# DRL-Navigation/DDRL4NAV

Measured on NVIDIA B200. Metric: PPO learner samples/s & batched policy actions/s at 1/2/4/8 B200, higher is better.
Workload: dtype f32 (three tcgen05 kind::f16 products of scaled fp16 hi/lo splits, fp32 accumulate)

## Files before the change

### ddrl4nav_b200/csrc/tc3.cu

```cuda
#include <cuda.h>
#include <cuda_fp16.h>

#include <algorithm>
#include <cstdlib>
#include <cstring>
#include <mutex>
#include <vector>

#include "common.cuh"
#include "layer_ops.h"
#include "prep_kernels.cuh"
#include "tc_ptx.cuh"

namespace ddrl {

constexpr int T3_BM = 128;
constexpr int T3_BK = 64;
constexpr int T3_CHUNK = 4;

__device__ unsigned long long g_tc3_wait[96];
#ifdef TC3_TIMING
#define T3_T0 const long long _t0 = clock64()
#define T3_ACC(acc) acc += clock64() - _t0
#define T3_WAIT(bar, par, acc) do { T3_T0; mbar_wait(bar, par); T3_ACC(acc); } while (0)
// ... 61 lines not shown
      ".reg .pred p;\n"
      "setp.ne.b32 p, %4, 0;\n"
      "tcgen05.mma.cta_group::1.kind::f16 [%0], [%1], %2, %3, p;\n"
      "}" ::"r"(tmem_d), "r"(tmem_a), "l"(db), "r"(idesc), "r"(accumulate) : "memory");
}

__device__ __forceinline__ void umma_f16_ss(uint32_t tmem_d, uint64_t da, uint64_t db, uint32_t idesc, uint32_t accumulate) {
  asm volatile(
      "{\n"
      ".reg .pred p;\n"
      "setp.ne.b32 p, %4, 0;\n"
      "tcgen05.mma.cta_group::1.kind::f16 [%0], %1, %2, %3, p;\n"
      "}" ::"r"(tmem_d), "l"(da), "l"(db), "r"(idesc), "r"(accumulate) : "memory");
}

template <int BN>
struct T3Cfg {
  static constexpr int A_SUB = T3_BM * 128;
  static constexpr int A_BYTES = 2 * A_SUB;
  static constexpr int B_BYTES = BN * 128;
  static constexpr int STAGE_BYTES = A_BYTES + 2 * B_BYTES;
  static constexpr int STAGES = BN <= 32 ? 5 : (BN <= 64 ? 4 : 3);
  static constexpr bool FOLD = BN <= 64;
  static constexpr int SA = BN <= 32 ? 4 : (BN <= 64 ? 3 : 2);
  static constexpr int NEPI = BN <= 32 ? 4 : 8;
  static constexpr int NSG = BN <= 64 ? 2 : 1;
  static constexpr int EPI0 = 4 + 4 * NSG;
  static constexpr int THREADS = (EPI0 + NEPI) * 32;
  static constexpr int COLS = BN / (NEPI / 4);
  static constexpr int TM_MAIN0 = 0, TM_MAIN1 = FOLD ? 2 * BN : BN, TM_CORR = FOLD ? 4 * BN : 2 * BN, TM_A = FOLD ? 5 * BN : 3 * BN;
  static constexpr int TMEM_COLS = 512;
  static constexpr int NBARS = 2 * STAGES + SA + 7;
  static constexpr int STG_OFF = STAGES * STAGE_BYTES;
  static constexpr int BAR_OFF = STG_OFF + NEPI * 4096;
  static constexpr int BIAS_OFF = BAR_OFF + 256;
  static constexpr int SMEM = 1024 + BIAS_OFF + BN * 4;
  static_assert(NBARS * 8 + 16 <= 256, "barrier block");
  static_assert(SMEM <= 232448, "shared memory budget");
  static_assert(TM_A + SA * 64 <= 512, "TMEM budget");
  static_assert(STAGES > SA, "the stage barrier of K block it - SA releases TMEM slot it % SA");
};

template <int BN>
__global__ void __launch_bounds__(T3Cfg<BN>::THREADS, 1)
tc3_kernel(const __grid_constant__ CUtensorMap tmA, const __grid_constant__ CUtensorMap tmBhi,
           const __grid_constant__ CUtensorMap tmBlo, const __grid_constant__ CUtensorMap tmA2,
           const __grid_constant__ CUtensorMap tmC, const __grid_constant__ CUtensorMap tmC2,
           const __grid_constant__ CUtensorMap tmM, const __grid_constant__ CUtensorMap tmM2, Tc3Args g) {
  using Cfg = T3Cfg<BN>;
  constexpr int S = Cfg::STAGES, SA = Cfg::SA;
  extern __shared__ uint8_t smem_dyn[];
  uint8_t* smem = smem_dyn + ((1024u - (smem_u32(smem_dyn) & 1023u)) & 1023u);
  uint64_t* bars = reinterpret_cast<uint64_t*>(smem + Cfg::BAR_OFF);
  uint64_t* bar_full = bars;
  uint64_t* bar_empty = bars + S;
  uint64_t* bar_aready = bars + 2 * S;
  uint64_t* bar_mfull = bars + 2 * S + SA;
  uint64_t* bar_mfree = bar_mfull + 2;
  uint64_t* bar_cfull = bar_mfull + 4;
  uint64_t* bar_cfree = bar_mfull + 5;
  uint64_t* bar_mask = bar_mfull + 6;
  uint32_t* tmem_slot = reinterpret_cast<uint32_t*>(bars + Cfg::NBARS);
  const int warp = threadIdx.x >> 5, lane = threadIdx.x & 31;
  const TcTap& tp = g.tap;
  const bool tapA = tp.mode != 0;

  if (warp == 0 && lane == 0) {
    mbar_init(smem_u32(bar_mask), 1);
    for (int s = 0; s < S; ++s) { mbar_init(smem_u32(bar_full + s), 1); mbar_init(smem_u32(bar_empty + s), 2); }
    for (int a = 0; a < SA; ++a) mbar_init(smem_u32(bar_aready + a), 4);
    for (int b = 0; b < 2; ++b) { mbar_init(smem_u32(bar_mfull + b), 1); mbar_init(smem_u32(bar_mfree + b), Cfg::NEPI); }
    mbar_init(smem_u32(bar_cfull), 1);
    mbar_init(smem_u32(bar_cfree), Cfg::NEPI);
    asm volatile("fence.mbarrier_init.release.cluster;" ::: "memory");
  }
  if (warp == 2) {
    asm volatile("tcgen05.alloc.cta_group::1.sync.aligned.shared::cta.b32 [%0], %1;" ::"r"(smem_u32(tmem_slot)),
                 "r"((uint32_t)Cfg::TMEM_COLS) : "memory");
    asm volatile("tcgen05.relinquish_alloc_permit.cta_group::1.sync.aligned;" ::: "memory");
  }
  tc_fence_before();
  __syncthreads();
  tc_fence_after();
  const uint32_t tmem_base = *tmem_slot;

  const int total_tiles = g.m_tiles * g.n_tiles;
  const int tile_step = (int)gridDim.x, tile_first = (int)blockIdx.x;
  const int nkb = g.kb_total;
  const bool ps = g.presplit != 0;
  const bool odd_tail = tapA && !ps && (tp.nslices & 1);

  if (warp == 0) {
    uint32_t it = 0;
    T3_ROLE_BEGIN
    for (int tile = tile_first; tile < total_tiles; tile += tile_step) {
      const int mt = tile / g.n_tiles, nt = tile - mt * g.n_tiles;
      const int m0 = mt * T3_BM, n0 = nt * BN;
      int b0 = 0, y0 = 0;
      const bool ph2 = tapA && mt >= tp.tiles1;
      if (tapA) {
        if (!ph2) { b0 = (mt / tp.tpi) * tp.nb; y0 = (mt % tp.tpi) * tp.ny * tp.sy - tp.py; }
        else { b0 = (mt - tp.tiles1) * tp.nb2; y0 = tp.y2 * tp.sy - tp.py; }
      }
      int cc = 0, kw = 0, kh = 0;
      for (int i = 0; i < nkb; ++i, ++it) {
        const uint32_t s = it % S;
        T3_WAITL(smem_u32(bar_empty + s), ((it / S) & 1) ^ 1, w0);
        const bool load_b = !g.b_resident || it < (uint32_t)S;
        const uint32_t b_tx = load_b ? 2u * Cfg::B_BYTES : 0u;
        if (elect_one()) {
          const uint32_t full = smem_u32(bar_full + s);
          const uint32_t a_dst = smem_u32(smem) + s * Cfg::STAGE_BYTES, bh_dst = a_dst + Cfg::A_BYTES, bl_dst = bh_dst + Cfg::B_BYTES;
          const int k = i * T3_BK;
          if (ps) {
            if (!tapA) {
              mbar_expect_tx(full, Cfg::A_BYTES + b_tx);
              tma_load_2d(&tmA, full, a_dst, k, m0);
              tma_load_2d(&tmM, full, a_dst + Cfg::A_SUB, k, m0);
            } else {
              const uint32_t box = (uint32_t)(ph2 ? tp.rows2 : tp.rows) * 128u;
              mbar_expect_tx(full, 2u * box + b_tx);
              tma_load_4d(ph2 ? &tmA2 : &tmA, full, a_dst, tp.c_off + cc * 64, kw - tp.px, y0 + kh, b0);
              tma_load_4d(ph2 ? &tmM2 : &tmM, full, a_dst + Cfg::A_SUB, tp.c_off + cc * 64, kw - tp.px, y0 + kh, b0);
            }
          } else if (!tapA) {
            mbar_expect_tx(full, Cfg::A_BYTES + b_tx);
            tma_load_2d(&tmA, full, a_dst, k, m0);
            tma_load_2d(&tmA, full, a_dst + Cfg::A_SUB, k + 32, m0);
          } else {
            const bool two = !(odd_tail && i == nkb - 1);
            const uint32_t box = (uint32_t)(ph2 ? tp.rows2 : tp.rows) * 128u;
            mbar_expect_tx(full, (two ? 2u : 1u) * box + b_tx);
            tma_load_4d(ph2 ? &tmA2 : &tmA, full, a_dst, tp.c_off + cc * 32, kw - tp.px, y0 + kh, b0);
            if (two) {
              int cc2 = cc + 1, kw2 = kw, kh2 = kh;
              if (cc2 == tp.cpb) { cc2 = 0; if (++kw2 == tp.KW) { kw2 = 0; ++kh2; } }
              tma_load_4d(ph2 ? &tmA2 : &tmA, full, a_dst + Cfg::A_SUB, tp.c_off + cc2 * 32, kw2 - tp.px, y0 + kh2, b0);
            }
          }
          if (load_b) {
            tma_load_2d(&tmBhi, full, bh_dst, k, n0);
            tma_load_2d(&tmBlo, full, bl_dst, k, n0);
          }
        }
        __syncwarp();
        if (tapA) {
#pragma unroll
          for (int j = 0; j < 2; ++j) {
            if (ps && j == 1) break;
            if (++cc == tp.cpb) { cc = 0; if (++kw == tp.KW) { kw = 0; ++kh; } }
          }
        }
      }
    }
    T3_ROLE_END(0, true);
  } else if (warp == 1 || warp == 3) {
    const bool chunk_role = warp == 1;
    const uint32_t idesc = (1u << 4) | ((uint32_t)(BN >> 3) << 17) | ((uint32_t)(T3_BM >> 4) << 24);
    const uint32_t idesc2 = (1u << 4) | ((uint32_t)((2 * BN) >> 3) << 17) | ((uint32_t)(T3_BM >> 4) << 24);
    const uint32_t smem_base = smem_u32(smem);
    const uint32_t t_corr = tmem_base + Cfg::TM_CORR;
    uint32_t it = 0, ch = 0, tl = 0;
    T3_ROLE_BEGIN
    for (int tile = tile_first; tile < total_tiles; tile += tile_step, ++tl) {
      for (int i = 0; i < nkb; ++i, ++it) {
        const uint32_t s = it % S, a = it % SA;
        const uint32_t buf = ch & 1;
        const bool first_in_chunk = (i % T3_CHUNK) == 0;
        const bool last_in_chunk = (i % T3_CHUNK) == T3_CHUNK - 1 || i == nkb - 1;
        const int ksteps = (odd_tail && i == nkb - 1) ? 2 : 4;
        if (chunk_role) { if (first_in_chunk) T3_WAIT(smem_u32(bar_mfree + buf), ((ch >> 1) & 1) ^ 1, w0); }
        else if (i == 0) T3_WAIT(smem_u32(bar_cfree), (tl & 1) ^ 1, w0);
        if (ps) T3_WAIT(smem_u32(bar_full + s), (it / S) & 1, w1);
        else T3_WAIT(smem_u32(bar_aready + a), (it / SA) & 1, w1);
        tc_fence_after();
        T3_SECTION_BEGIN;
        if (elect_one()) {
          const uint32_t b_hi = smem_base + s * Cfg::STAGE_BYTES + Cfg::A_BYTES, b_lo = b_hi + Cfg::B_BYTES;
          const uint32_t a_hi = tmem_base + Cfg::TM_A + a * 64, a_lo = a_hi + 32;
          const uint64_t dbh0 = umma_desc(b_hi, 16, 1024, 2);
          if (ps) {
            const uint32_t sa_hi = smem_base + s * Cfg::STAGE_BYTES;
            const uint64_t dah0 = umma_desc(sa_hi, 16, 1024, 2), dal0 = umma_desc(sa_hi + Cfg::A_SUB, 16, 1024, 2);
            if (chunk_role) {
              const uint32_t t_main = tmem_base + (buf ? Cfg::TM_MAIN1 : Cfg::TM_MAIN0);
#pragma unroll
              for (int k4 = 0; k4 < 4; ++k4)
                umma_f16_ss(t_main, dah0 + k4 * 2, dbh0 + k4 * 2, Cfg::FOLD ? idesc2 : idesc, (!first_in_chunk || k4 != 0) ? 1u : 0u);
              umma_commit(smem_u32(bar_empty + s));
              if (last_in_chunk) umma_commit(smem_u32(bar_mfull + buf));
            } else {
              const uint64_t dbl0 = umma_desc(b_lo, 16, 1024, 2);
#pragma unroll
              for (int k4 = 0; k4 < 4; ++k4) {
                umma_f16_ss(t_corr, dal0 + k4 * 2, dbh0 + k4 * 2, idesc, (i | k4) != 0 ? 1u : 0u);
                if (!Cfg::FOLD) umma_f16_ss(t_corr, dah0 + k4 * 2, dbl0 + k4 * 2, idesc, 1u);
              }
              umma_commit(smem_u32(bar_empty + s));
              if (i == nkb - 1) umma_commit(smem_u32(bar_cfull));
            }
          } else if (chunk_role) {
            const uint32_t t_main = tmem_base + (buf ? Cfg::TM_MAIN1 : Cfg::TM_MAIN0);
#pragma unroll
            for (int k4 = 0; k4 < 4; ++k4) {
              if (k4 >= ksteps) break;
              umma_f16_ts(t_main, a_hi + k4 * 8, dbh0 + k4 * 2, Cfg::FOLD ? idesc2 : idesc, (!first_in_chunk || k4 != 0) ? 1u : 0u);
            }
            umma_commit(smem_u32(bar_empty + s));
            if (last_in_chunk) umma_commit(smem_u32(bar_mfull + buf));
          } else {
            const uint64_t dbl0 = umma_desc(b_lo, 16, 1024, 2);
#pragma unroll
            for (int k4 = 0; k4 < 4; ++k4) {
              if (k4 >= ksteps) break;
              umma_f16_ts(t_corr, a_lo + k4 * 8, dbh0 + k4 * 2, idesc, (i | k4) != 0 ? 1u : 0u);
              if (!Cfg::FOLD) umma_f16_ts(t_corr, a_hi + k4 * 8, dbl0 + k4 * 2, idesc, 1u);
            }
            umma_commit(smem_u32(bar_empty + s));
            if (i == nkb - 1) umma_commit(smem_u32(bar_cfull));
          }
        }
        __syncwarp();
        T3_SECTION_END(w2);
        if (last_in_chunk) ++ch;
      }
    }
    T3_ROLE_END(chunk_role ? 1 : 2, true);
  } else if (warp >= 4 && warp < Cfg::EPI0) {
    const int q = (warp - 4) & 3, grp = (warp - 4) >> 2;
    const uint32_t t_lane = (uint32_t)(q * 32) << 16;
    float sA, sA_inv;
    t3_scale(__ldg(g.amax_a), sA, sA_inv);
    const bool unit_scale = sA == 1.f;
    const int row = q * 32 + lane;
// ... 32 lines not shown
            }
          }
          if (j == 0) {
            if (it >= (uint32_t)SA) {
              const uint32_t jj = it - SA;
              T3_WAIT(smem_u32(bar_empty + (jj % S)), (jj / S) & 1, w1);
            }
            tc_fence_after();
          }
          tmem_st16(ta + j * 16, hi);
          tmem_st16(ta + 32 + j * 16, lo);
        }
        asm volatile("tcgen05.wait::st.sync.aligned;" ::: "memory");
        tc_fence_before();
        __syncwarp();
        if (lane == 0) mbar_arrive(smem_u32(bar_aready + a));
        T3_SECTION_END(w2);
      }
    }
    T3_ROLE_END(3, warp == 4);
  } else if (warp == 2) {
    if (g.tma_store) {
      const bool masked = g.tma_mask != 0;
      const bool fusedT = tapA && tp.ncls > 1;
      for (int tile = tile_first; tile < total_tiles; tile += tile_step) {
        const int mt = tile / g.n_tiles, nt = tile - mt * g.n_tiles;
        const int m0 = mt * T3_BM, n0 = nt * BN;
        int cy = 0, cb = 0;
        const bool ph2 = tapA && mt >= tp.tiles1;
        if (tapA) {
          cb = ph2 ? (mt - tp.tiles1) * tp.nb2 : (mt / tp.tpi) * tp.nb;
          cy = ph2 ? tp.y2 : (mt % tp.tpi) * tp.ny;
        }
        const uint32_t box_bytes = tapA ? (uint32_t)(ph2 ? tp.rows2 : tp.rows) * 128u : 16384u;
        auto coords = [&](int col, int& c0, int& c1, int& c2, int& c3) {
          c0 = col; c1 = 0; c2 = cy; c3 = cb;
          if (fusedT) {
            const int qq = col / tp.cls_cols;
            c0 = col - qq * tp.cls_cols; c1 = tp.cls_ix[qq]; c2 = tp.out_s * cy + tp.cls_iy[qq];
          }
        };
// ... 61 lines not shown
    float s_pre = 1.f, s_out = sA_inv * sB_inv;
    if (!(s_out >= 1e-30f && s_out <= 1e30f)) { s_pre = sA_inv; s_out = sB_inv; }
    const int r = q * 32 + lane;
    int ryb1 = 0, ryb2 = 0;
    const bool need_off = !g.tma_store || g.bits_out != nullptr || g.bits_in != nullptr;
    const int rx = (tapA && need_off) ? r % tp.Xn : 0;
    if (tapA) {
      const int t1 = r / tp.Xn;
      ryb1 = (t1 % tp.ny) | ((t1 / tp.ny) << 16);
      if (tp.ny2 > 0) ryb2 = (t1 % tp.ny2) | ((t1 / tp.ny2) << 16);
    }
    float* bias_s = reinterpret_cast<float*>(smem + Cfg::BIAS_OFF);
    const int et = e * 32 + lane;
    T3_ROLE_BEGIN
    for (int tile = tile_first; tile < total_tiles; tile += tile_step, ++tl) {
      const int mt = tile / g.n_tiles, nt = tile - mt * g.n_tiles;
      const int m0 = mt * T3_BM, n0 = nt * BN;
      int cy = 0, cb = 0;
      if (tapA) {
        const bool ph2 = mt >= tp.tiles1;
        cb = ph2 ? (mt - tp.tiles1) * tp.nb2 : (mt / tp.tpi) * tp.nb;
        cy = ph2 ? tp.y2 : (mt % tp.tpi) * tp.ny;
      }
      const bool masked = g.tma_store && g.tma_mask;
      float bias_r = 0.f;
      if (g.tma_store && et < BN && g.bias != nullptr && n0 + et < g.N) bias_r = __ldg(g.bias + n0 + et);
      const bool ph2e = tapA && mt >= tp.tiles1;
      const int ryb = ph2e ? ryb2 : ryb1;
      const bool rvalid = tapA ? (r < (ph2e ? tp.rows2 : tp.rows) && cb + (ryb >> 16) < tp.Bn && cy + (ryb & 0xffff) < tp.Yn)
                               : (m0 + r) < g.M;
      const bool fused = tapA && tp.ncls > 1;
// ... 25 lines not shown
          }
          if (inb) mw[p] = __ldg(g.bits_in + (eoff >> 5));
        }
      }
      float acc[Cfg::COLS];
#pragma unroll
      for (int j = 0; j < Cfg::COLS; ++j) acc[j] = 0.f;
      const int nch = (nkb + T3_CHUNK - 1) / T3_CHUNK;
      for (int c = 0; c < nch; ++c, ++ch) {
        const int buf = ch & 1;
        T3_WAITL(smem_u32(bar_mfull + buf), (ch >> 1) & 1, w0);
        tc_fence_after();
#pragma unroll
        for (int j0 = 0; j0 < Cfg::COLS; j0 += 32) {
          float v[32];
          if (Cfg::FOLD && c == 0) {
            tmem_ld32x2(tmem_base + t_lane + (buf ? Cfg::TM_MAIN1 : Cfg::TM_MAIN0) + col0 + j0,
                        tmem_base + t_lane + (buf ? Cfg::TM_MAIN1 : Cfg::TM_MAIN0) + BN + col0 + j0, acc + j0, v);
#pragma unroll
            for (int j = 0; j < 32; ++j) acc[j0 + j] = fmaf(v[j], T3_LO_INV, acc[j0 + j]);
            continue;
          }
          tmem_ld32(tmem_base + t_lane + (buf ? Cfg::TM_MAIN1 : Cfg::TM_MAIN0) + col0 + j0, v);
#pragma unroll
          for (int j = 0; j < 32; ++j) acc[j0 + j] += v[j];
          if (Cfg::FOLD) {
            tmem_ld32(tmem_base + t_lane + (buf ? Cfg::TM_MAIN1 : Cfg::TM_MAIN0) + BN + col0 + j0, v);
#pragma unroll
            for (int j = 0; j < 32; ++j) acc[j0 + j] = fmaf(v[j], T3_LO_INV, acc[j0 + j]);
          }
        }
        tc_fence_before();
        __syncwarp();
        if (lane == 0) mbar_arrive(smem_u32(bar_mfree + buf));
      }
      T3_WAITL(smem_u32(bar_cfull), tl & 1, w1);
      tc_fence_after();
#pragma unroll
      for (int j0 = 0; j0 < Cfg::COLS; j0 += 32) {
        float v[32];
        tmem_ld32(tmem_base + t_lane + Cfg::TM_CORR + col0 + j0, v);
#pragma unroll
        for (int j = 0; j < 32; ++j) acc[j0 + j] = fmaf(v[j], T3_LO_INV, acc[j0 + j]);
      }
      tc_fence_before();
      __syncwarp();
      if (lane == 0) mbar_arrive(smem_u32(bar_cfree));
      if (s_pre != 1.f) {
#pragma unroll
        for (int j = 0; j < Cfg::COLS; ++j) acc[j] *= s_pre;
      }
      T3_SECTION_BEGIN;
      const float neg_slope = g.act == 3 ? 0.f : 0.01f;
      if (!g.tma_store) {
#pragma unroll
        for (int j = 0; j < Cfg::COLS; ++j) acc[j] *= s_out;
      }
      if (g.tma_store) {
        float* stg = reinterpret_cast<float*>(smem + Cfg::STG_OFF) + e * 1024;
        const bool relu = g.act == 1;
        const float slope = g.act == 2 ? 0.01f : 1.f;
        const bool has_bias = g.bias != nullptr;
// ... 210 lines not shown
              }
            }
          }
        }
      }
      T3_SECTION_END(w2);
    }
    T3_ROLE_END(4, warp == Cfg::EPI0);
    if (g.amax_out != nullptr) {
#pragma unroll
      for (int o = 16; o > 0; o >>= 1) run_max = fmaxf(run_max, __shfl_xor_sync(0xffffffffu, run_max, o));
      if (lane == 0 && run_max > 0.f) atomicMax(reinterpret_cast<unsigned int*>(g.amax_out), __float_as_uint(run_max));
    }
  }
  tc_fence_before();
  __syncthreads();
  if (warp == 2) {
    asm volatile("tcgen05.dealloc.cta_group::1.sync.aligned.b32 %0, %1;" ::"r"(tmem_base), "r"((uint32_t)Cfg::TMEM_COLS)
                 : "memory");
  }
}

struct Tc3Maps { CUtensorMap a, bhi, blo, a2, c, c2, m, m2; };

template <int BN>
static int launch3(const Tc3Maps& m, const Tc3Args& g, dim3 grid, cudaStream_t s) {
  using Cfg = T3Cfg<BN>;
  static bool attr_done_dev[64] = {};
  bool& attr_done = attr_done_dev[current_device_index()];
  if (!attr_done) {
    DDRL_CUDA(cudaFuncSetAttribute(tc3_kernel<BN>, cudaFuncAttributeMaxDynamicSharedMemorySize, Cfg::SMEM));
    attr_done = true;
  }
  static const bool no_bres = [] { const char* e = getenv("DDRL_TC3_NO_BRES"); return e && e[0] == '1'; }();
  Tc3Args ga = g;
  ga.b_resident = (!no_bres && g.n_tiles == 1 && g.kb_total >= 1 && Cfg::STAGES % g.kb_total == 0) ? 1 : 0;
  tc3_kernel<BN><<<grid, Cfg::THREADS, Cfg::SMEM, s>>>(m.a, m.bhi, m.blo, m.a2, m.c, m.c2, m.m, m.m2, ga);
  prof_work(2.0 * g.M * (double)g.N * g.K * (g.tap.work_scale > 0.f ? g.tap.work_scale : 1.f));
  if (g_prof_on && g_prof_shapes) {
    char nm[96];
    snprintf(nm, sizeof(nm), "%s3[fwd,M=%d,N=%d,K=%d,g=%d]", g.tap.mode ? "conv_tc" : "gemm_tc", g.M, g.N, g.K,
             (int)(grid.x * grid.y * grid.z));
    DDRL_LAUNCHED(prof_intern(nm));
    return DDRL_OK;
  }
  DDRL_LAUNCHED("tc3_kernel");
  return DDRL_OK;
}

static int launch3_bn(int bn, const Tc3Maps& m, const Tc3Args& g, dim3 grid, cudaStream_t s) {
  switch (bn) {
    case 128: return launch3<128>(m, g, grid, s);
    case 64: return launch3<64>(m, g, grid, s);
    default: return launch3<32>(m, g, grid, s);
  }
}
static const bool g_t3_tma_store = [] { const char* e = getenv("DDRL_TC3_TMA_STORE"); return !(e && e[0] == '0'); }();
static const bool g_t3_tma_dgrad = [] { const char* e = getenv("DDRL_TC3_TMA_DGRAD"); return !(e && e[0] == '0'); }();

static inline int pick_bn3(int N) { return N > 64 ? 128 : (N > 32 ? 64 : 32); }
static inline bool al16(const void* p) { return (reinterpret_cast<uintptr_t>(p) & 15) == 0; }

static int make_map_b16(CUtensorMap* m, const void* base, int K, int N, int ldb16, int bn) {
  const unsigned long long dims[2] = {(unsigned long long)K, (unsigned long long)N};
  const unsigned long long strides[1] = {(unsigned long long)ldb16 * 2};
  const unsigned box[2] = {64u, (unsigned)bn}, estr[2] = {1u, 1u};
  return tc_encode_tiled(m, true, 2, base, dims, strides, box, estr, true);
}

// ... 70 lines not shown
  if (M < 1 || N < 1 || K < 1) return false;
  if (!al16(A) || !al16(Bhi) || !al16(Blo) || lda % 4 != 0 || ldb16 % 8 != 0) return false;
  return true;
}

int tc3_gemm(int M, int N, int K, const float* A, int lda, const void* Bhi, const void* Blo, int ldb16, const float* amax_a,
             const float* amax_b, float* C, int ldc, const float* bias, int act, const float* mask, float* amax_out,
             cudaStream_t s) {
  if (!tc3_gemm_supported(M, N, K, A, lda, Bhi, Blo, ldb16)) return DDRL_E_UNSUPPORTED;
  if ((act >= 3 && !mask) || !amax_a || !amax_b) return DDRL_E_ARG;
  int r = tc_get_encode();
  if (r != DDRL_OK) return r;
  const int bn = pick_bn3(N);
  Tc3Maps mp;
  r = tc_make_map(&mp.a, A, K, M, lda, T3_BM, false);
  if (r == DDRL_OK) r = make_map_b16(&mp.bhi, Bhi, K, N, ldb16, bn);
  if (r == DDRL_OK) r = make_map_b16(&mp.blo, Blo, K, N, ldb16, bn);
  if (r != DDRL_OK) return r;
  mp.a2 = mp.a;
  Tc3Args g;
  memset(&g, 0, sizeof(g));
  g.C = C; g.bias = bias; g.mask = mask; g.act = act;
  g.M = M; g.N = N; g.K = K; g.sCm = ldc; g.sCn = 1;
  g.kb_total = ceil_div(K, T3_BK); g.kb_per_split = g.kb_total;
  g.m_tiles = ceil_div(M, T3_BM); g.n_tiles = ceil_div(N, bn);
  g.amax_a = amax_a; g.amax_b = amax_b; g.amax_out = amax_out;
  g.vec_store = (ldc % 4 == 0 && al16(C) && (!mask || al16(mask))) ? 1 : 0;
  const bool tma_ok = g.vec_store && g_t3_tma_store && (act < 3 || g_t3_tma_dgrad);
  const unsigned int* mbits = (tma_ok && act >= 3 && ldc % 32 == 0) ? signbits_for_mask(mask) : nullptr;
  if (tma_ok) {
    const unsigned long long dims[2] = {(unsigned long long)N, (unsigned long long)M};
    const unsigned long long strides[1] = {(unsigned long long)ldc * 4};
    const unsigned box[2] = {32u, (unsigned)T3_BM}, estr[2] = {1u, 1u};
    int rs = tc_encode_tiled(&mp.c, false, 2, C, dims, strides, box, estr, true);
    if (rs == DDRL_OK && act >= 3 && !mbits) rs = tc_encode_tiled(&mp.m, false, 2, mask, dims, strides, box, estr, true);
    if (rs == DDRL_OK) { g.tma_store = 1; g.tma_mask = (act >= 3 && !mbits) ? 1 : 0; g.bits_in = mbits; }
  }
  g.bits_out = signbits_for_output(C, g.tma_store && (act == 1 || act == 2) && ldc == N && N % 32 == 0);
  if (!g.tma_store) mp.c = mp.a;
  mp.c2 = mp.c;
  if (!g.tma_mask) mp.m = mp.c;
  mp.m2 = mp.m;
  dim3 grid(std::min(g.m_tiles * g.n_tiles, kNumSMs), 1, 1);
  return launch3_bn(bn, mp, g, grid, s);
}

int tc3_conv_fwd(const ConvOp& o, const void* Whi, const void* Wlo, int ldw16, int N, const float* amax_a, const float* amax_b,
                 const float* bias, int act, const float* mask, float* out, long long osb, long long osy, long long osx,
                 float* amax_out, cudaStream_t s, const TcTap* cls, const void* a_hi16, const void* a_lo16) {
  if (!conv_tc_supported(o, false) || N < 1 || ldw16 % 8 != 0 || !al16(Whi) || !al16(Wlo)) return DDRL_E_UNSUPPORTED;
  if ((act >= 3 && !mask) || !amax_a || !amax_b) return DDRL_E_ARG;
  const bool ps = a_hi16 != nullptr || a_lo16 != nullptr;
  if (ps && (!presplit_ok(o, a_hi16, a_lo16) || act >= 3)) return DDRL_E_UNSUPPORTED;
  int r = tc_get_encode();
  if (r != DDRL_OK) return r;
  const int bn = pick_bn3(N);
  Tc3Args g;
  memset(&g, 0, sizeof(g));
  tc_tap_common(g.tap, o, T3_BM, true);
// ... 7 lines not shown
      if (cls->cls_off[q] % 4 != 0) return DDRL_E_ARG;
    }
  }
  const int K = o.KH * o.KW * o.Cin;
  Tc3Maps mp;
  const bool ph2 = g.tap.ny2 > 0;
  if (ps) {
    g.presplit = 1;
    g.tap.cpb = o.Cin / 64; g.tap.nslices = o.KH * o.KW * g.tap.cpb;
    r = make_map_nhwc16(&mp.a, a_hi16, o, o.Xn, g.tap.ny, g.tap.nb);
    if (r == DDRL_OK && ph2) r = make_map_nhwc16(&mp.a2, a_hi16, o, o.Xn, g.tap.ny2, g.tap.nb2);
  } else {
    r = tc_make_map_nhwc(&mp.a, o, o.Xn, g.tap.ny, g.tap.nb, false);
    if (r == DDRL_OK && ph2) r = tc_make_map_nhwc(&mp.a2, o, o.Xn, g.tap.ny2, g.tap.nb2, false);
  }
  if (r == DDRL_OK) r = make_map_b16(&mp.bhi, Whi, K, N, ldw16, bn);
  if (r == DDRL_OK) r = make_map_b16(&mp.blo, Wlo, K, N, ldw16, bn);
  if (r != DDRL_OK) return r;
  if (!ph2) mp.a2 = mp.a;
  g.C = out; g.bias = bias; g.mask = mask; g.act = act;
  g.M = o.Bn * o.Yn * o.Xn; g.N = N; g.K = K; g.sCm = 0; g.sCn = 1;
  g.kb_total = ps ? g.tap.nslices : (g.tap.nslices + 1) / 2; g.kb_per_split = g.kb_total;
  g.m_tiles = ceil_div(o.Bn, g.tap.nb) * g.tap.tpi + (ph2 ? ceil_div(o.Bn, g.tap.nb2) : 0);
  g.n_tiles = ceil_div(N, bn);
  g.amax_a = amax_a; g.amax_b = amax_b; g.amax_out = amax_out;
  g.vec_store = (osb % 4 == 0 && osy % 4 == 0 && osx % 4 == 0 && al16(out) && (!mask || al16(mask))) ? 1 : 0;
  const bool classes = g.tap.ncls > 1;
  const long long ct = classes && g.tap.out_s > 0 ? osx / g.tap.out_s : 0;
  const bool classes_ok = classes && g_t3_tma_dgrad && g.tap.cls_cols % 32 == 0 && g.tap.out_W > 1 && g.tap.ncls == g.tap.out_s * g.tap.out_s &&
                          ct > 0 && osx == ct * g.tap.out_s && osy == (long long)g.tap.out_s * g.tap.out_W * ct &&
                          osb == (long long)g.tap.out_H * g.tap.out_W * ct;
  const bool tma_ok = g.vec_store && g_t3_tma_store && (act < 3 || g_t3_tma_dgrad) && (!classes || classes_ok);
// ... 18 lines not shown
    }
    if (rs == DDRL_OK) { g.tma_store = 1; g.tma_mask = (act >= 3 && !mbits) ? 1 : 0; g.bits_in = mbits; }
  }
  g.bits_out = signbits_for_output(out, g.tma_store && !classes && (act == 1 || act == 2) && N % 32 == 0 && osx == N &&
                                            osy == (long long)o.Xn * N && osb == (long long)o.Yn * o.Xn * N);
  if (!g.tma_store) mp.c = mp.a;
  if (!g.tma_store || !ph2) mp.c2 = mp.c;
  if (!g.tma_mask) mp.m = mp.c;
  if (!g.tma_mask || !ph2) mp.m2 = mp.m;
  if (ps) {
    r = make_map_nhwc16(&mp.m, a_lo16, o, o.Xn, g.tap.ny, g.tap.nb);
    if (r == DDRL_OK && ph2) r = make_map_nhwc16(&mp.m2, a_lo16, o, o.Xn, g.tap.ny2, g.tap.nb2);
    if (r != DDRL_OK) return r;
    if (!ph2) mp.m2 = mp.m;
  }
  dim3 grid(std::min(g.m_tiles * g.n_tiles, kNumSMs), 1, 1);
  return launch3_bn(bn, mp, g, grid, s);
}

template <int BN>
struct T3WCfg {
  static_assert(BN == 64 || BN == 128, "weight-gradient tiles are 64 or 128 columns");
  static constexpr int R_SUB = T3_BK * 128;
  static constexpr int A_SUB = R_SUB;
  static constexpr int A_BYTES = 4 * A_SUB;
  static constexpr int BRAW_BYTES = (BN / 32) * R_SUB;
  static constexpr int STAGE_BYTES = A_BYTES + BRAW_BYTES;
  static constexpr int B16_TILE = T3_BK * 128;
  static constexpr int B16_BYTES = 2 * (BN / 64) * B16_TILE;
  static constexpr bool FOLD = BN <= 64;
  static constexpr int SA = BN <= 64 ? 3 : 2;
  static constexpr int STAGES = BN <= 64 ? 3 : 2;
// ... 624 lines not shown
```

### ddrl4nav_b200/csrc/tc_ptx.cuh

```cuda
#pragma once
#include <cuda.h>
#include <cuda_runtime.h>
#include <stdint.h>

#include "layer_ops.h"

namespace ddrl {

__device__ __forceinline__ uint32_t smem_u32(const void* p) { return (uint32_t)__cvta_generic_to_shared(p); }

__device__ __forceinline__ void mbar_init(uint32_t bar, uint32_t count) {
  asm volatile("mbarrier.init.shared::cta.b64 [%0], %1;" ::"r"(bar), "r"(count));
}
__device__ __forceinline__ void mbar_expect_tx(uint32_t bar, uint32_t bytes) {
  asm volatile("mbarrier.arrive.expect_tx.shared::cta.b64 _, [%0], %1;" ::"r"(bar), "r"(bytes) : "memory");
}
__device__ __forceinline__ void mbar_arrive(uint32_t bar) {
  asm volatile("mbarrier.arrive.shared::cta.b64 _, [%0];" ::"r"(bar) : "memory");
}
__device__ __forceinline__ void mbar_wait(uint32_t bar, uint32_t parity) {
  asm volatile(
      "{\n"
      ".reg .pred P1;\n"
      "LAB_WAIT:\n"
// ... 125 lines not shown
      "{\n"
      ".reg .pred p, e;\n"
      "setp.ne.b32 e, %5, 0;\n"
      "setp.ne.b32 p, %4, 0;\n"
      "@e tcgen05.mma.cta_group::1.kind::tf32 [%0], [%1], %2, %3, p;\n"
      "}" ::"r"(tmem_d), "r"(tmem_a), "l"(db), "r"(idesc), "r"(accumulate), "r"(leader) : "memory");
}
__device__ __forceinline__ void umma_commit_lead(uint32_t leader, uint32_t bar) {
  asm volatile(
      "{\n"
      ".reg .pred e;\n"
      "setp.ne.b32 e, %1, 0;\n"
      "@e tcgen05.commit.cta_group::1.mbarrier::arrive::one.shared::cluster.b64 [%0];\n"
      "}" ::"r"(bar), "r"(leader) : "memory");
}
__device__ __forceinline__ void tmem_st16(uint32_t taddr, const uint32_t* r) {
  asm volatile(
      "tcgen05.st.sync.aligned.32x32b.x16.b32 [%0], {%1,%2,%3,%4,%5,%6,%7,%8,%9,%10,%11,%12,%13,%14,%15,%16};"
      ::"r"(taddr), "r"(r[0]), "r"(r[1]), "r"(r[2]), "r"(r[3]), "r"(r[4]), "r"(r[5]), "r"(r[6]), "r"(r[7]), "r"(r[8]),
        "r"(r[9]), "r"(r[10]), "r"(r[11]), "r"(r[12]), "r"(r[13]), "r"(r[14]), "r"(r[15]) : "memory");
}

int tc_get_encode();
int tc_make_map(CUtensorMap* m, const float* base, long long inner, long long outer, long long ld, int box_outer, bool mn_major);
int tc_encode_tiled(CUtensorMap* m, bool f16, int rank, const void* base, const unsigned long long* dims,
                    const unsigned long long* strides_bytes, const unsigned* box, const unsigned* estr, int swizzle);
int tc_make_map_nhwc(CUtensorMap* m, const ConvOp& o, int nx, int ny, int nb, bool mn_major);
int tc_make_map_dy4(CUtensorMap* m, const float* dy, int ldy, int N, int Xn, int Yn, int Bn, int xw, int yh);
int tc_make_map_dy3(CUtensorMap* m, const float* dy, int ldy, int N, long long ipix, int Bn, int rows);
void tc_tap_common(TcTap& t, const ConvOp& o, int cap, bool two_phase = false);
// ... 3 lines not shown
```

Baseline: 1.730 million.

## Add 2-CTA paired tcgen05 MMA path for tc3 GEMM/conv kernels

Adds a cluster-of-two variant of the tc3 kernel. It uses cta_group::2 tcgen05 MMA with an M=256 tile spread across two CTAs, and each CTA loads half of the B tile. Only rank 0 issues MMAs. Commits are multicast to both CTAs, and the epilogue and A-staging barriers arrive across the cluster. The goal is to halve B-operand shared-memory traffic and use the larger pair MMA. The cost is cluster synchronisation and a new, unverified barrier protocol. The path is enabled by default for BN>=64 when the kernel is not presplit, B is not resident, and there are at least two M tiles.

```diff
diff --git a/ddrl4nav_b200/csrc/tc3.cu b/ddrl4nav_b200/csrc/tc3.cu
--- a/ddrl4nav_b200/csrc/tc3.cu
+++ b/ddrl4nav_b200/csrc/tc3.cu
@@ -99,6 +99,30 @@
       "}" ::"r"(tmem_d), "l"(da), "l"(db), "r"(idesc), "r"(accumulate) : "memory");
 }
 
+__device__ __forceinline__ void umma_f16_ts_pair(uint32_t tmem_d, uint32_t tmem_a, uint64_t db, uint32_t idesc, uint32_t accumulate) {
+  asm volatile(
+      "{\n"
+      ".reg .pred p;\n"
+      "setp.ne.b32 p, %4, 0;\n"
+      "tcgen05.mma.cta_group::2.kind::f16 [%0], [%1], %2, %3, p;\n"
+      "}" ::"r"(tmem_d), "r"(tmem_a), "l"(db), "r"(idesc), "r"(accumulate) : "memory");
+}
+template <bool PAIR>
+__device__ __forceinline__ void t3_mma_ts(uint32_t tmem_d, uint32_t tmem_a, uint64_t db, uint32_t idesc, uint32_t accumulate) {
+  if (PAIR) umma_f16_ts_pair(tmem_d, tmem_a, db, idesc, accumulate);
+  else umma_f16_ts(tmem_d, tmem_a, db, idesc, accumulate);
+}
+template <bool PAIR>
+__device__ __forceinline__ void t3_commit(uint32_t bar) {
+  if (PAIR) umma_commit_pair(bar);
+  else umma_commit(bar);
+}
+template <bool PAIR>
+__device__ __forceinline__ void t3_arrive_issuer(uint32_t bar) {
+  if (PAIR) mbar_arrive_cluster(mapa_shared(bar, 0));
+  else mbar_arrive(bar);
+}
+
 template <int BN>
 struct T3Cfg {
   static constexpr int A_SUB = T3_BM * 128;
@@ -126,7 +150,7 @@
   static_assert(STAGES > SA, "the stage barrier of K block it - SA releases TMEM slot it % SA");
 };
 
-template <int BN>
+template <int BN, bool PAIR>
 __global__ void __launch_bounds__(T3Cfg<BN>::THREADS, 1)
 tc3_kernel(const __grid_constant__ CUtensorMap tmA, const __grid_constant__ CUtensorMap tmBhi,
            const __grid_constant__ CUtensorMap tmBlo, const __grid_constant__ CUtensorMap tmA2,
@@ -149,37 +173,53 @@
   const int warp = threadIdx.x >> 5, lane = threadIdx.x & 31;
   const TcTap& tp = g.tap;
   const bool tapA = tp.mode != 0;
+  const int rank = PAIR ? (int)(blockIdx.x & 1) : 0;
 
   if (warp == 0 && lane == 0) {
+    constexpr uint32_t NC = PAIR ? 2 : 1;
     mbar_init(smem_u32(bar_mask), 1);
     for (int s = 0; s < S; ++s) { mbar_init(smem_u32(bar_full + s), 1); mbar_init(smem_u32(bar_empty + s), 2); }
-    for (int a = 0; a < SA; ++a) mbar_init(smem_u32(bar_aready + a), 4);
-    for (int b = 0; b < 2; ++b) { mbar_init(smem_u32(bar_mfull + b), 1); mbar_init(smem_u32(bar_mfree + b), Cfg::NEPI); }
+    for (int a = 0; a < SA; ++a) mbar_init(smem_u32(bar_aready + a), 4 * NC);
+    for (int b = 0; b < 2; ++b) { mbar_init(smem_u32(bar_mfull + b), 1); mbar_init(smem_u32(bar_mfree + b), Cfg::NEPI * NC); }
     mbar_init(smem_u32(bar_cfull), 1);
-    mbar_init(smem_u32(bar_cfree), Cfg::NEPI);
+    mbar_init(smem_u32(bar_cfree), Cfg::NEPI * NC);
     asm volatile("fence.mbarrier_init.release.cluster;" ::: "memory");
   }
   if (warp == 2) {
-    asm volatile("tcgen05.alloc.cta_group::1.sync.aligned.shared::cta.b32 [%0], %1;" ::"r"(smem_u32(tmem_slot)),
-                 "r"((uint32_t)Cfg::TMEM_COLS) : "memory");
-    asm volatile("tcgen05.relinquish_alloc_permit.cta_group::1.sync.aligned;" ::: "memory");
+    if (PAIR) {
+      asm volatile("tcgen05.alloc.cta_group::2.sync.aligned.shared::cta.b32 [%0], %1;" ::"r"(smem_u32(tmem_slot)),
+                   "r"((uint32_t)Cfg::TMEM_COLS) : "memory");
+      asm volatile("tcgen05.relinquish_alloc_permit.cta_group::2.sync.aligned;" ::: "memory");
+    } else {
+      asm volatile("tcgen05.alloc.cta_group::1.sync.aligned.shared::cta.b32 [%0], %1;" ::"r"(smem_u32(tmem_slot)),
+                   "r"((uint32_t)Cfg::TMEM_COLS) : "memory");
+      asm volatile("tcgen05.relinquish_alloc_permit.cta_group::1.sync.aligned;" ::: "memory");
+    }
   }
   tc_fence_before();
-  __syncthreads();
+  if (PAIR) cluster_sync();
+  else __syncthreads();
   tc_fence_after();
   const uint32_t tmem_base = *tmem_slot;
 
-  const int total_tiles = g.m_tiles * g.n_tiles;
+  const int total_tiles = PAIR ? 2 * (((g.m_tiles + 1) >> 1) * g.n_tiles) : g.m_tiles * g.n_tiles;
   const int tile_step = (int)gridDim.x, tile_first = (int)blockIdx.x;
+  auto t3_mtile = [&](int tile, int& mt, int& nt) {
+    const int pt = PAIR ? tile >> 1 : tile;
+    const int mp = pt / g.n_tiles;
+    nt = pt - mp * g.n_tiles;
+    mt = PAIR ? 2 * mp + (tile & 1) : mp;
+  };
   const int nkb = g.kb_total;
-  const bool ps = g.presplit != 0;
+  const bool ps = !PAIR && g.presplit != 0;
   const bool odd_tail = tapA && !ps && (tp.nslices & 1);
 
   if (warp == 0) {
     uint32_t it = 0;
     T3_ROLE_BEGIN
     for (int tile = tile_first; tile < total_tiles; tile += tile_step) {
-      const int mt = tile / g.n_tiles, nt = tile - mt * g.n_tiles;
+      int mt, nt;
+      t3_mtile(tile, mt, nt);
       const int m0 = mt * T3_BM, n0 = nt * BN;
       int b0 = 0, y0 = 0;
       const bool ph2 = tapA && mt >= tp.tiles1;
@@ -192,10 +232,11 @@
         const uint32_t s = it % S;
         T3_WAITL(smem_u32(bar_empty + s), ((it / S) & 1) ^ 1, w0);
         const bool load_b = !g.b_resident || it < (uint32_t)S;
-        const uint32_t b_tx = load_b ? 2u * Cfg::B_BYTES : 0u;
+        constexpr uint32_t B_LD = PAIR ? Cfg::B_BYTES / 2 : Cfg::B_BYTES;
+        const uint32_t b_tx = load_b ? 2u * B_LD : 0u;
         if (elect_one()) {
           const uint32_t full = smem_u32(bar_full + s);
-          const uint32_t a_dst = smem_u32(smem) + s * Cfg::STAGE_BYTES, bh_dst = a_dst + Cfg::A_BYTES, bl_dst = bh_dst + Cfg::B_BYTES;
+          const uint32_t a_dst = smem_u32(smem) + s * Cfg::STAGE_BYTES, bh_dst = a_dst + Cfg::A_BYTES, bl_dst = bh_dst + B_LD;
           const int k = i * T3_BK;
           if (ps) {
             if (!tapA) {
@@ -224,8 +265,9 @@
             }
           }
           if (load_b) {
-            tma_load_2d(&tmBhi, full, bh_dst, k, n0);
-            tma_load_2d(&tmBlo, full, bl_dst, k, n0);
+            const int nb0 = PAIR ? n0 + rank * (BN / 2) : n0;
+            tma_load_2d(&tmBhi, full, bh_dst, k, nb0);
+            tma_load_2d(&tmBlo, full, bl_dst, k, nb0);
           }
         }
         __syncwarp();
@@ -239,10 +281,11 @@
       }
     }
     T3_ROLE_END(0, true);
-  } else if (warp == 1 || warp == 3) {
+  } else if ((warp == 1 || warp == 3) && rank == 0) {
     const bool chunk_role = warp == 1;
-    const uint32_t idesc = (1u << 4) | ((uint32_t)(BN >> 3) << 17) | ((uint32_t)(T3_BM >> 4) << 24);
-    const uint32_t idesc2 = (1u << 4) | ((uint32_t)((2 * BN) >> 3) << 17) | ((uint32_t)(T3_BM >> 4) << 24);
+    constexpr uint32_t MM = PAIR ? 2 * T3_BM : T3_BM;
+    const uint32_t idesc = (1u << 4) | ((uint32_t)(BN >> 3) << 17) | ((uint32_t)(MM >> 4) << 24);
+    const uint32_t idesc2 = (1u << 4) | ((uint32_t)((2 * BN) >> 3) << 17) | ((uint32_t)(MM >> 4) << 24);
     const uint32_t smem_base = smem_u32(smem);
     const uint32_t t_corr = tmem_base + Cfg::TM_CORR;
     uint32_t it = 0, ch = 0, tl = 0;
@@ -261,7 +304,7 @@
         tc_fence_after();
         T3_SECTION_BEGIN;
         if (elect_one()) {
-          const uint32_t b_hi = smem_base + s * Cfg::STAGE_BYTES + Cfg::A_BYTES, b_lo = b_hi + Cfg::B_BYTES;
+          const uint32_t b_hi = smem_base + s * Cfg::STAGE_BYTES + Cfg::A_BYTES, b_lo = b_hi + (PAIR ? Cfg::B_BYTES / 2 : Cfg::B_BYTES);
           const uint32_t a_hi = tmem_base + Cfg::TM_A + a * 64, a_lo = a_hi + 32;
           const uint64_t dbh0 = umma_desc(b_hi, 16, 1024, 2);
           if (ps) {
@@ -289,20 +332,20 @@
 #pragma unroll
             for (int k4 = 0; k4 < 4; ++k4) {
               if (k4 >= ksteps) break;
-              umma_f16_ts(t_main, a_hi + k4 * 8, dbh0 + k4 * 2, Cfg::FOLD ? idesc2 : idesc, (!first_in_chunk || k4 != 0) ? 1u : 0u);
-            }
-            umma_commit(smem_u32(bar_empty + s));
-            if (last_in_chunk) umma_commit(smem_u32(bar_mfull + buf));
+              t3_mma_ts<PAIR>(t_main, a_hi + k4 * 8, dbh0 + k4 * 2, Cfg::FOLD ? idesc2 : idesc, (!first_in_chunk || k4 != 0) ? 1u : 0u);
+            }
+            t3_commit<PAIR>(smem_u32(bar_empty + s));
+            if (last_in_chunk) t3_commit<PAIR>(smem_u32(bar_mfull + buf));
           } else {
             const uint64_t dbl0 = umma_desc(b_lo, 16, 1024, 2);
 #pragma unroll
             for (int k4 = 0; k4 < 4; ++k4) {
               if (k4 >= ksteps) break;
-              umma_f16_ts(t_corr, a_lo + k4 * 8, dbh0 + k4 * 2, idesc, (i | k4) != 0 ? 1u : 0u);
-              if (!Cfg::FOLD) umma_f16_ts(t_corr, a_hi + k4 * 8, dbl0 + k4 * 2, idesc, 1u);
-            }
-            umma_commit(smem_u32(bar_empty + s));
-            if (i == nkb - 1) umma_commit(smem_u32(bar_cfull));
+              t3_mma_ts<PAIR>(t_corr, a_lo + k4 * 8, dbh0 + k4 * 2, idesc, (i | k4) != 0 ? 1u : 0u);
+              if (!Cfg::FOLD) t3_mma_ts<PAIR>(t_corr, a_hi + k4 * 8, dbl0 + k4 * 2, idesc, 1u);
+            }
+            t3_commit<PAIR>(smem_u32(bar_empty + s));
+            if (i == nkb - 1) t3_commit<PAIR>(smem_u32(bar_cfull));
           }
         }
         __syncwarp();
@@ -365,7 +408,7 @@
         asm volatile("tcgen05.wait::st.sync.aligned;" ::: "memory");
         tc_fence_before();
         __syncwarp();
-        if (lane == 0) mbar_arrive(smem_u32(bar_aready + a));
+        if (lane == 0) t3_arrive_issuer<PAIR>(smem_u32(bar_aready + a));
         T3_SECTION_END(w2);
       }
     }
@@ -375,7 +418,8 @@
       const bool masked = g.tma_mask != 0;
       const bool fusedT = tapA && tp.ncls > 1;
       for (int tile = tile_first; tile < total_tiles; tile += tile_step) {
-        const int mt = tile / g.n_tiles, nt = tile - mt * g.n_tiles;
+        int mt, nt;
+        t3_mtile(tile, mt, nt);
         const int m0 = mt * T3_BM, n0 = nt * BN;
         int cy = 0, cb = 0;
         const bool ph2 = tapA && mt >= tp.tiles1;
@@ -467,7 +511,8 @@
     const int et = e * 32 + lane;
     T3_ROLE_BEGIN
     for (int tile = tile_first; tile < total_tiles; tile += tile_step, ++tl) {
-      const int mt = tile / g.n_tiles, nt = tile - mt * g.n_tiles;
+      int mt, nt;
+      t3_mtile(tile, mt, nt);
       const int m0 = mt * T3_BM, n0 = nt * BN;
       int cy = 0, cb = 0;
       if (tapA) {
@@ -523,25 +568,27 @@
 #pragma unroll
         for (int j0 = 0; j0 < Cfg::COLS; j0 += 32) {
           float v[32];
+          const uint32_t mc = PAIR && Cfg::FOLD ? 2 * (col0 + j0) : col0 + j0;
+          const uint32_t cc = PAIR && Cfg::FOLD ? mc + 32 : BN + col0 + j0;
           if (Cfg::FOLD && c == 0) {
-            tmem_ld32x2(tmem_base + t_lane + (buf ? Cfg::TM_MAIN1 : Cfg::TM_MAIN0) + col0 + j0,
-                        tmem_base + t_lane + (buf ? Cfg::TM_MAIN1 : Cfg::TM_MAIN0) + BN + col0 + j0, acc + j0, v);
+            tmem_ld32x2(tmem_base + t_lane + (buf ? Cfg::TM_MAIN1 : Cfg::TM_MAIN0) + mc,
+                        tmem_base + t_lane + (buf ? Cfg::TM_MAIN1 : Cfg::TM_MAIN0) + cc, acc + j0, v);
 #pragma unroll
             for (int j = 0; j < 32; ++j) acc[j0 + j] = fmaf(v[j], T3_LO_INV, acc[j0 + j]);
             continue;
           }
-          tmem_ld32(tmem_base + t_lane + (buf ? Cfg::TM_MAIN1 : Cfg::TM_MAIN0) + col0 + j0, v);
+          tmem_ld32(tmem_base + t_lane + (buf ? Cfg::TM_MAIN1 : Cfg::TM_MAIN0) + mc, v);
 #pragma unroll
           for (int j = 0; j < 32; ++j) acc[j0 + j] += v[j];
           if (Cfg::FOLD) {
-            tmem_ld32(tmem_base + t_lane + (buf ? Cfg::TM_MAIN1 : Cfg::TM_MAIN0) + BN + col0 + j0, v);
+            tmem_ld32(tmem_base + t_lane + (buf ? Cfg::TM_MAIN1 : Cfg::TM_MAIN0) + cc, v);
 #pragma unroll
             for (int j = 0; j < 32; ++j) acc[j0 + j] = fmaf(v[j], T3_LO_INV, acc[j0 + j]);
           }
         }
         tc_fence_before();
         __syncwarp();
-        if (lane == 0) mbar_arrive(smem_u32(bar_mfree + buf));
+        if (lane == 0) t3_arrive_issuer<PAIR>(smem_u32(bar_mfree + buf));
       }
       T3_WAITL(smem_u32(bar_cfull), tl & 1, w1);
       tc_fence_after();
@@ -554,7 +601,7 @@
       }
       tc_fence_before();
       __syncwarp();
-      if (lane == 0) mbar_arrive(smem_u32(bar_cfree));
+      if (lane == 0) t3_arrive_issuer<PAIR>(smem_u32(bar_cfree));
       if (s_pre != 1.f) {
 #pragma unroll
         for (int j = 0; j < Cfg::COLS; ++j) acc[j] *= s_pre;
@@ -795,28 +842,68 @@
     }
   }
   tc_fence_before();
-  __syncthreads();
+  if (PAIR) cluster_sync();
+  else __syncthreads();
   if (warp == 2) {
-    asm volatile("tcgen05.dealloc.cta_group::1.sync.aligned.b32 %0, %1;" ::"r"(tmem_base), "r"((uint32_t)Cfg::TMEM_COLS)
-                 : "memory");
+    if (PAIR)
+      asm volatile("tcgen05.dealloc.cta_group::2.sync.aligned.b32 %0, %1;" ::"r"(tmem_base), "r"((uint32_t)Cfg::TMEM_COLS)
+                   : "memory");
+    else
+      asm volatile("tcgen05.dealloc.cta_group::1.sync.aligned.b32 %0, %1;" ::"r"(tmem_base), "r"((uint32_t)Cfg::TMEM_COLS)
+                   : "memory");
   }
 }
 
 struct Tc3Maps { CUtensorMap a, bhi, blo, a2, c, c2, m, m2; };
 
-template <int BN>
-static int launch3(const Tc3Maps& m, const Tc3Args& g, dim3 grid, cudaStream_t s) {
+static const bool g_t3_no_bres = [] { const char* e = getenv("DDRL_TC3_NO_BRES"); return e && e[0] == '1'; }();
+static int t3_stages(int bn) { return bn == 128 ? T3Cfg<128>::STAGES : (bn == 64 ? T3Cfg<64>::STAGES : T3Cfg<32>::STAGES); }
+static bool t3_resident(int bn, const Tc3Args& g) {
+  return !g_t3_no_bres && g.n_tiles == 1 && g.kb_total >= 1 && t3_stages(bn) % g.kb_total == 0;
+}
+static bool t3_pair(int bn, const Tc3Args& g) {
+  const char* e = getenv("DDRL_TC3_NO_PAIR");
+  if (e && e[0] == '1') return false;
+  return bn >= 64 && !g.presplit && !t3_resident(bn, g) && g.m_tiles >= 2;
+}
+
+template <int BN, bool PAIR>
+static int launch3(const Tc3Maps& m, const Tc3Args& g, cudaStream_t s) {
   using Cfg = T3Cfg<BN>;
   static bool attr_done_dev[64] = {};
-  bool& attr_done = attr_done_dev[current_device_index()];
-  if (!attr_done) {
-    DDRL_CUDA(cudaFuncSetAttribute(tc3_kernel<BN>, cudaFuncAttributeMaxDynamicSharedMemorySize, Cfg::SMEM));
-    attr_done = true;
-  }
-  static const bool no_bres = [] { const char* e = getenv("DDRL_TC3_NO_BRES"); return e && e[0] == '1'; }();
+  static int pairs_dev[64] = {};
+  const int dev = current_device_index();
+  if (!attr_done_dev[dev]) {
+    DDRL_CUDA(cudaFuncSetAttribute(tc3_kernel<BN, PAIR>, cudaFuncAttributeMaxDynamicSharedMemorySize, Cfg::SMEM));
+    if (PAIR) {
+      cudaLaunchConfig_t cfg = {};
+      cudaLaunchAttribute at[1];
+      at[0].id = cudaLaunchAttributeClusterDimension;
+      at[0].val.clusterDim.x = 2; at[0].val.clusterDim.y = 1; at[0].val.clusterDim.z = 1;
+      cfg.gridDim = dim3(2 * (kNumSMs / 2), 1, 1); cfg.blockDim = dim3(Cfg::THREADS, 1, 1); cfg.dynamicSmemBytes = Cfg::SMEM;
+      cfg.attrs = at; cfg.numAttrs = 1;
+      int n = 0;
+      DDRL_CUDA(cudaOccupancyMaxActiveClusters(&n, tc3_kernel<BN, PAIR>, &cfg));
+      if (n < 1) return DDRL_E_UNSUPPORTED;
+      pairs_dev[dev] = n;
+    }
+    attr_done_dev[dev] = true;
+  }
   Tc3Args ga = g;
-  ga.b_resident = (!no_bres && g.n_tiles == 1 && g.kb_total >= 1 && Cfg::STAGES % g.kb_total == 0) ? 1 : 0;
-  tc3_kernel<BN><<<grid, Cfg::THREADS, Cfg::SMEM, s>>>(m.a, m.bhi, m.blo, m.a2, m.c, m.c2, m.m, m.m2, ga);
+  ga.b_resident = (!PAIR && t3_resident(BN, g)) ? 1 : 0;
+  const int tiles = (PAIR ? (g.m_tiles + 1) / 2 : g.m_tiles) * g.n_tiles;
+  const dim3 grid(PAIR ? 2 * std::min(tiles, pairs_dev[dev]) : std::min(tiles, kNumSMs), 1, 1);
+  if (PAIR) {
+    cudaLaunchConfig_t cfg = {};
+    cudaLaunchAttribute at[1];
+    at[0].id = cudaLaunchAttributeClusterDimension;
+    at[0].val.clusterDim.x = 2; at[0].val.clusterDim.y = 1; at[0].val.clusterDim.z = 1;
+    cfg.gridDim = grid; cfg.blockDim = dim3(Cfg::THREADS, 1, 1); cfg.dynamicSmemBytes = Cfg::SMEM; cfg.stream = s;
+    cfg.attrs = at; cfg.numAttrs = 1;
+    cudaLaunchKernelEx(&cfg, tc3_kernel<BN, PAIR>, m.a, m.bhi, m.blo, m.a2, m.c, m.c2, m.m, m.m2, ga);
+  } else {
+    tc3_kernel<BN, PAIR><<<grid, Cfg::THREADS, Cfg::SMEM, s>>>(m.a, m.bhi, m.blo, m.a2, m.c, m.c2, m.m, m.m2, ga);
+  }
   prof_work(2.0 * g.M * (double)g.N * g.K * (g.tap.work_scale > 0.f ? g.tap.work_scale : 1.f));
   if (g_prof_on && g_prof_shapes) {
     char nm[96];
@@ -829,11 +916,12 @@
   return DDRL_OK;
 }
 
-static int launch3_bn(int bn, const Tc3Maps& m, const Tc3Args& g, dim3 grid, cudaStream_t s) {
+static int launch3_bn(int bn, bool pair, const Tc3Maps& m, const Tc3Args& g, cudaStream_t s) {
+  if (pair) return bn == 128 ? launch3<128, true>(m, g, s) : launch3<64, true>(m, g, s);
   switch (bn) {
-    case 128: return launch3<128>(m, g, grid, s);
-    case 64: return launch3<64>(m, g, grid, s);
-    default: return launch3<32>(m, g, grid, s);
+    case 128: return launch3<128, false>(m, g, s);
+    case 64: return launch3<64, false>(m, g, s);
+    default: return launch3<32, false>(m, g, s);
   }
 }
 static const bool g_t3_tma_store = [] { const char* e = getenv("DDRL_TC3_TMA_STORE"); return !(e && e[0] == '0'); }();
@@ -934,8 +1022,6 @@
   const int bn = pick_bn3(N);
   Tc3Maps mp;
   r = tc_make_map(&mp.a, A, K, M, lda, T3_BM, false);
-  if (r == DDRL_OK) r = make_map_b16(&mp.bhi, Bhi, K, N, ldb16, bn);
-  if (r == DDRL_OK) r = make_map_b16(&mp.blo, Blo, K, N, ldb16, bn);
   if (r != DDRL_OK) return r;
   mp.a2 = mp.a;
   Tc3Args g;
@@ -961,8 +1047,11 @@
   mp.c2 = mp.c;
   if (!g.tma_mask) mp.m = mp.c;
   mp.m2 = mp.m;
-  dim3 grid(std::min(g.m_tiles * g.n_tiles, kNumSMs), 1, 1);
-  return launch3_bn(bn, mp, g, grid, s);
+  const bool pair = t3_pair(bn, g);
+  r = make_map_b16(&mp.bhi, Bhi, K, N, ldb16, pair ? bn / 2 : bn);
+  if (r == DDRL_OK) r = make_map_b16(&mp.blo, Blo, K, N, ldb16, pair ? bn / 2 : bn);
+  if (r != DDRL_OK) return r;
+  return launch3_bn(bn, pair, mp, g, s);
 }
 
 int tc3_conv_fwd(const ConvOp& o, const void* Whi, const void* Wlo, int ldw16, int N, const float* amax_a, const float* amax_b,
@@ -1000,8 +1089,6 @@
     r = tc_make_map_nhwc(&mp.a, o, o.Xn, g.tap.ny, g.tap.nb, false);
     if (r == DDRL_OK && ph2) r = tc_make_map_nhwc(&mp.a2, o, o.Xn, g.tap.ny2, g.tap.nb2, false);
   }
-  if (r == DDRL_OK) r = make_map_b16(&mp.bhi, Whi, K, N, ldw16, bn);
-  if (r == DDRL_OK) r = make_map_b16(&mp.blo, Wlo, K, N, ldw16, bn);
   if (r != DDRL_OK) return r;
   if (!ph2) mp.a2 = mp.a;
   g.C = out; g.bias = bias; g.mask = mask; g.act = act;
@@ -1050,8 +1137,11 @@
     if (r != DDRL_OK) return r;
     if (!ph2) mp.m2 = mp.m;
   }
-  dim3 grid(std::min(g.m_tiles * g.n_tiles, kNumSMs), 1, 1);
-  return launch3_bn(bn, mp, g, grid, s);
+  const bool pair = t3_pair(bn, g);
+  r = make_map_b16(&mp.bhi, Whi, K, N, ldw16, pair ? bn / 2 : bn);
+  if (r == DDRL_OK) r = make_map_b16(&mp.blo, Wlo, K, N, ldw16, pair ? bn / 2 : bn);
+  if (r != DDRL_OK) return r;
+  return launch3_bn(bn, pair, mp, g, s);
 }
 
 template <int BN>
diff --git a/ddrl4nav_b200/csrc/tc_ptx.cuh b/ddrl4nav_b200/csrc/tc_ptx.cuh
--- a/ddrl4nav_b200/csrc/tc_ptx.cuh
+++ b/ddrl4nav_b200/csrc/tc_ptx.cuh
@@ -163,6 +163,22 @@
       "@e tcgen05.commit.cta_group::1.mbarrier::arrive::one.shared::cluster.b64 [%0];\n"
       "}" ::"r"(bar), "r"(leader) : "memory");
 }
+__device__ __forceinline__ void cluster_sync() {
+  asm volatile("barrier.cluster.arrive.release.aligned;\nbarrier.cluster.wait.acquire.aligned;" ::: "memory");
+}
+__device__ __forceinline__ uint32_t mapa_shared(uint32_t addr, uint32_t rank) {
+  uint32_t r;
+  asm volatile("mapa.shared::cluster.u32 %0, %1, %2;" : "=r"(r) : "r"(addr), "r"(rank));
+  return r;
+}
+__device__ __forceinline__ void mbar_arrive_cluster(uint32_t cluster_addr) {
+  asm volatile("mbarrier.arrive.shared::cluster.b64 _, [%0];" ::"r"(cluster_addr) : "memory");
+}
+__device__ __forceinline__ void umma_commit_pair(uint32_t bar) {
+  asm volatile("tcgen05.commit.cta_group::2.mbarrier::arrive::one.shared::cluster.multicast::cluster.b64 [%0], %1;"
+               ::"r"(bar), "h"((uint16_t)3) : "memory");
+}
+
 __device__ __forceinline__ void tmem_st16(uint32_t taddr, const uint32_t* r) {
   asm volatile(
       "tcgen05.st.sync.aligned.32x32b.x16.b32 [%0], {%1,%2,%3,%4,%5,%6,%7,%8,%9,%10,%11,%12,%13,%14,%15,%16};"
```

Result: faster. 1.758 million (median of 6 runs) (+1.6%).
